# SayanoAI/Comfy-RVC

Hardware: AMD Instinct MI355X
Metric: audio-sec/wall-sec (xRT), 40k_v2 end-to-end VC (higher is better)
Workload: dtype f32; 1 GPU; Full VC 40k_v2 (HuBERT -> RMVPE -> SynthesizerTrnMs768NSFsid), 30 s 16 kHz clips, 12 per GPU per step (3 in flight), vc_single host array in -> int16 host array out (BASELINE.json configs[2]); clips_in_flight_per_gpu=3, weights=procedural (comfy-rvc_amd/synthetic.py), noise=device generator, seeded per clip, parallelism=clip-per-GPU x1 (3 lanes each), one RCCL gather of the step's int16 waveforms

## Files before the change

### comfy-rvc_amd/_lib.py

```python
import ctypes as C
import os

_HERE = os.path.dirname(os.path.abspath(__file__))
LIB_PATH = os.environ.get("RVC_HIP_LIB") or os.path.join(_HERE, "csrc", "librvc_hip.so")


class RvcHipError(RuntimeError):
    pass


def _load():
    if not os.path.isfile(LIB_PATH):
        raise RvcHipError(
            f"{LIB_PATH} is missing: build it with `python -c 'import __graft_entry__ as g; g.build()'` "
            "(or `make -C comfy-rvc_amd/csrc`).  There is no CPU fallback.")
    return C.CDLL(LIB_PATH)


lib = _load()

c_void_p, c_int, c_int64, c_float, c_char_p = C.c_void_p, C.c_int, C.c_int64, C.c_float, C.c_char_p
P = C.POINTER


# ... 148 lines not shown
    "rvc_spectrogram_batch_ms": (c_int, [c_void_p, c_void_p, c_void_p, c_int64, c_void_p, c_int, c_int, c_int, c_float, c_int, c_void_p, c_int64]),
    "rvc_multiscale_mel_loss": (c_int, [c_void_p, c_void_p, c_int, P(c_void_p), P(c_int64), P(c_int64), c_int, c_int64, P(C.c_int32), P(C.c_int32), c_int, c_int,
                                        c_void_p]),
    "rvc_hpss": (c_int, [c_void_p, c_void_p, c_int, c_int, c_int, c_void_p, c_void_p, c_int]),
    "rvc_hpss_l1": (c_int, [c_void_p, c_void_p, c_void_p, c_int, c_int, c_int, c_float, c_void_p]),
    "rvc_tsi_terms": (c_int, [c_void_p, c_void_p, c_void_p, c_int, c_int, c_int, c_float, c_void_p]),
    "rvc_op_gemm_split": (c_int, [c_void_p] * 7 + [c_int] * 4 + [c_float, c_int, c_float] + [c_int] * 5),
    "rvc_op_conv2d_split": (c_int, [c_void_p] * 7 + [c_int] * 9),
    "rvc_op_wn_in_gate_split": (c_int, [c_void_p] * 6 + [c_int] * 4),
    "rvc_op_gemm_split_qkv": (c_int, [c_void_p] * 6 + [c_int] * 4),
    "rvc_op_conv1d_s2_split": (c_int, [c_void_p] * 6 + [c_int] * 5),
    "rvc_op_conv1d_split": (c_int, [c_void_p] * 6 + [c_int] * 9),
    "rvc_op_conv1d": (c_int, [c_void_p, c_void_p, c_void_p, c_void_p, c_void_p, c_void_p] + [c_int] * 8 +
                      [c_int, c_float, c_int, c_float, c_int, c_float, c_int]),
    "rvc_op_conv_transpose1d": (c_int, [c_void_p, c_void_p, c_void_p, c_void_p, c_void_p] + [c_int] * 6 + [c_int, c_float, c_int]),
    "rvc_op_conv2d3x3": (c_int, [c_void_p, c_void_p, c_void_p, c_void_p, c_void_p, c_void_p] + [c_int] * 5),
    "rvc_op_conv_transpose2d": (c_int, [c_void_p, c_void_p, c_void_p, c_void_p, c_void_p] + [c_int] * 5),
    "rvc_op_gemm_tn": (c_int, [c_void_p, c_void_p, c_void_p, c_void_p] + [c_int] * 4),
    "rvc_conv1d_plan_create": (c_int, [c_void_p, c_void_p] + [c_int] * 7 + [P(c_void_p)]),
    "rvc_conv1d_plan_run": (c_int, [c_void_p, c_void_p, c_void_p, c_int, c_void_p, c_void_p, c_int, c_float, c_int, c_float]),
    "rvc_conv1d_plan_pair_run": (c_int, [c_void_p, c_void_p, c_void_p, c_void_p, c_int, c_void_p, c_float, c_int]),
    "rvc_conv1d_plan_resblock_run": (c_int, [P(c_void_p), c_void_p, c_void_p, c_int, c_void_p, c_float, c_int, P(c_int), c_void_p, c_void_p, c_void_p]),
    "rvc_conv1d_plan_pair_split_run": (c_int, [c_void_p, c_void_p, c_void_p, c_void_p, c_int, c_void_p, c_float, c_int]),
    "rvc_conv1d_plan_destroy": (c_int, [c_void_p]),
    "rvc_op_attention": (c_int, [c_void_p, c_void_p, c_void_p, c_void_p, c_void_p, c_void_p, c_int, c_int]),
    "rvc_op_attention_split": (c_int, [c_void_p] * 7 + [c_int, c_int]),
    "rvc_op_attention_split_rel": (c_int, [c_void_p] * 9 + [c_int, c_int, c_int]),
    "rvc_op_cbr2_small": (c_int, [c_void_p] * 7 + [c_int, c_int, c_int]),
    "rvc_op_layernorm_c_split": (c_int, [c_void_p] * 6 + [c_int, c_int]),
    "rvc_op_conv3_small": (c_int, [c_void_p] * 7 + [c_int] * 6),
# ... 100 lines not shown
```

### comfy-rvc_amd/csrc/conv_kernels.h

```cpp
#pragma once
#include "rvc_internal.h"
#include <hip/hip_ext.h>

namespace rvc {

typedef float f32x16 __attribute__((ext_vector_type(16)));
typedef unsigned int u32x4 __attribute__((ext_vector_type(4)));

struct ConvArgsX : ConvArgs {
  long long ldW;
  int Wcols;
  int Wrows;
  int ksplit; float* partial; long long ldP;
  unsigned magRP, magPW;
  int ni; unsigned magNI;
  const unsigned char* Wx; int CoPx; int xbufs; int NC; int kreal; long long wxBatch;
  const unsigned char* Wx2; const float* bias1; int fuse_p2; float fuse_slope;
  const unsigned char* Xs; long long xsTp;
  unsigned char* Ys; long long ysTp; float ys_slope;
  int wbufs;
  int xcd_remap;
  int h2;
};

__device__ __forceinline__ __amdgpu_buffer_rsrc_t make_rsrc(const void* base, unsigned bytes) {
  return __builtin_amdgcn_make_buffer_rsrc(const_cast<void*>(base), 0, (int)bytes, 0x00020000);
}
constexpr unsigned kOOB = 0x80000000u;
__device__ __forceinline__ float buf_load(__amdgpu_buffer_rsrc_t r, unsigned voff, unsigned soff = 0) {
  return __uint_as_float(__builtin_amdgcn_raw_buffer_load_b32(r, (int)voff, (int)soff, 0));
}
__device__ __forceinline__ void buf_dma(__amdgpu_buffer_rsrc_t rs, unsigned char* lds_dst, int voffset, int soffset) {
  __builtin_amdgcn_raw_ptr_buffer_load_lds(rs, (__attribute__((address_space(3))) void*)lds_dst, 16, voffset, soffset, 0, 0);
}

template <int WM, int WN, int AM, int AN, int G, bool HAS_R, bool HAS_ACC>
__device__ __forceinline__ void dense_epilogue_t(const ConvArgsX& p, f32x16 (&acc)[AM][AN], int z, int co0, int n0, int wm, int wn, int li, int lh) {
// ... 104 lines not shown
  dim3 grid; size_t lds = 0;
  int prof_cfg = 0, prof_fused = 0;
  double alg_bytes = 0.0, flops = 0.0;
};
bool conv_x3_plan(const ConvArgsX& a0, int batch, long long Tplan, ConvPlan& p);
void conv_plan_launch(const ConvPlan& p, hipStream_t s);
bool conv_x3p_plan(ConvPlan& p, int AM, int AN);
int conv_x3p_check_read();
bool conv_x3q_plan(ConvPlan& p, int AM, int AN);
bool conv_x3g_plan(ConvPlan& p);
bool conv_x3pf_plan(ConvPlan& p);
bool conv_rbh_plan(ConvPlan& p);
bool conv_x3_pair_plan(const ConvLayer& c1, const ConvLayer& c2, const float* X, long long ldX, int T, long long Tplan, float* Y, long long ldY,
                       const ConvEpilogue& e2, int h2, ConvPlan& p);

struct Rb3Args {
  const float* X; long long ldX; float* Y; long long ldY;
  const unsigned char* W[6];
  const float* B[6];
  int CoPx;
  int T, halo, NO;
  float pre_slope, mid_slope, out_scale;
  const float* nsrc; const float* nw; const float* nb;
};
struct Rb3Plan {
  Rb3Args a; void (*launch)(const Rb3Args&, dim3, size_t, hipStream_t) = nullptr; dim3 grid; size_t lds = 0;
  int C = 0, k = 0, accumulate = 0;
};
bool conv_rb3_plan(const ConvLayer* const* c1, const ConvLayer* const* c2, const float* X, long long ldX, int T, long long Tplan, float* Y, long long ldY,
                   float pre_slope, float out_scale, int accumulate, int h2, const float* nsrc, const float* nw, const float* nb, Rb3Plan& p);
// ... 4 lines not shown
```

### comfy-rvc_amd/csrc/conv_mfma.hip

```cpp
#include "conv_kernels.h"
#include "phase_timing.h"
#include <atomic>
#include <tuple>

#ifndef RVC_EPI_TWOPHASE
#define RVC_EPI_TWOPHASE 0
#endif

namespace rvc {

RVC_PHASE_TABLE_REGISTER;

constexpr int kWSlots = 32;
__host__ __device__ constexpr int x_slots(int BN, int MODE) {
  return MODE == 2 ? (BN >= 512 ? 26 : (BN >= 256 ? 18 : 14)) : (BN >= 512 ? 36 : (BN >= 256 ? 20 : (BN >= 128 ? 32 : 16)));
}

template <int WM, int WN, int AM, int AN, int MODE>
__global__ __launch_bounds__(256) void conv_mfma_kernel(const ConvArgsX p) {
  constexpr int BM = WM * AM * 32, BN = WN * AN * 32;
  constexpr int XS = x_slots(BN, MODE);
  extern __shared__ __attribute__((aligned(16))) float smem[];
  const int CK = p.CK, WROW = p.WROW;
  float* Xs = smem;
// ... 504 lines not shown
          const int u = tap / stride, r = tap % stride;
          const int vc = ci * stride + r;
          const int chunk = vc / L.CK, vcc = vc % L.CK;
          P[(size_t)g * L.wBatch + (((size_t)chunk * L.ktaps + u) * L.CK + vcc) * L.CoP + co] =
              w[((size_t)(g * Cog + co) * Cig + ci) * k + tap];
        }
  upload_layer(L, P, bias, Co);
  if ((g_precision == 2 || (g_precision == 1 && g_x3_default)) && groups == 1 && Ci % 16 == 0 && Co >= 32) {
    pack_x3(L, w, Co, Ci, k);
    if (stride == 1 && Ci == Co && (k == 3 || k == 7 || k == 11) && ((Co % 64 == 0 && Ci >= 64) || Co == 32) && pad == dil * (k - 1) / 2) pack_h2(L, w, Co, Ci, k);
  }
  if ((g_precision == 2 || (g_precision == 1 && g_x3_default)) && groups > 1 && stride == 1 && Cig % 16 == 0 && Cog % 16 == 0 && dil >= 1)
    pack_x3_grouped(L, w, groups, Cog, Cig, k);
}

void tconv1d_layer_init(ConvLayer& L, const float* w, const float* bias, int Ci, int Co, int k, int u, int pad) {
  const int E2 = (k - 1 - pad) / u, E1 = (u - 1 + pad) / u;
  L.mode = 1; L.groups = 1; L.Ci = Ci; L.co_real = Co; L.Co = u * Co; L.CoP = (L.Co + 31) & ~31;
  L.k = E1 + E2 + 1; L.stride = 1; L.dil = 1; L.pad = E2; L.tconv_u = u; L.up2 = 0;
  L.ktaps = L.k;
  L.CK = pick_ck(Ci, L.ktaps, 1);
  L.nchunk = (Ci + L.CK - 1) / L.CK;
  L.wBatch = (long long)L.nchunk * L.ktaps * L.CK * L.CoP;
  std::vector<float> P((size_t)L.wBatch, 0.f);
  for (int r = 0; r < u; ++r)
    for (int co = 0; co < Co; ++co)
      for (int ci = 0; ci < Ci; ++ci)
        for (int j = 0; j < L.ktaps; ++j) {
          const int e = E2 - j;
          const int kk = e * u + r + pad;
          if (kk < 0 || kk >= k) continue;
          const int chunk = ci / L.CK, vcc = ci % L.CK;
          P[(((size_t)chunk * L.ktaps + j) * L.CK + vcc) * L.CoP + (size_t)co * u + r] = w[((size_t)ci * Co + co) * k + kk];
        }
  if ((g_precision == 2 || (g_precision == 1 && g_x3_default)) && Ci % 16 == 0 && L.Co >= 32) {
    std::vector<float> Weq((size_t)L.Co * Ci * L.ktaps, 0.f);
    for (int r = 0; r < u; ++r)
      for (int co = 0; co < Co; ++co)
        for (int ci = 0; ci < Ci; ++ci)
          for (int j = 0; j < L.ktaps; ++j) {
            const int kk = (E2 - j) * u + r + pad;
            if (kk >= 0 && kk < k) Weq[(((size_t)co * u + r) * Ci + ci) * L.ktaps + j] = w[((size_t)ci * Co + co) * k + kk];
          }
    pack_x3(L, Weq.data(), L.Co, Ci, L.ktaps);
  }
  L.k = k; L.pad = pad;
  L.dil = 1;
  L.conv_pad = E2;
  upload_layer(L, P, bias, Co);
}

void conv2d_kx_layer_init(ConvLayer& L, const float* w, const float* bias, int Co, int Ci, int KH, int KW, int PH, int PWL) {
  RVC_REQUIRE(Ci % 16 == 0 && KH >= 1 && KW >= 1 && PH >= 0 && PH < KH && PWL >= 0 && PWL < KW, "conv2d_kx: Ci must be a multiple of 16, padding inside the window");
  L.mode = 2; L.groups = 1; L.Ci = Ci; L.Co = Co; L.co_real = Co; L.CoP = (Co + 31) & ~31;
  L.k = KH * KW; L.stride = 1; L.dil = 1; L.pad = 0; L.tconv_u = 0; L.up2 = 0; L.ktaps = KH * KW;
  L.kh = KH; L.kw = KW; L.ph = PH; L.pwl = PWL;
  L.CK = 16; L.nchunk = Ci / 16; L.wBatch = 0;
  pack_x3(L, w, Co, Ci, KH * KW);
  L.bd_ = bias ? dev_upload(bias, Co) : nullptr;
}
// ... 147 lines not shown
  ProfRec r{t.a, t.b, flops, cfg, bytes, 0, 0, 0, 0, 0, 0, 0, 1, fused, blocks, 0};
  if (a) { r.h2 = a->h2; r.Ci = a->Ci; r.Co = a->Co; r.k = a->kreal > 0 ? a->kreal : a->ktaps; r.dil = a->dil; r.stride = a->stride; r.Tout = a->Tout; r.Wd = a->Wd; r.ksplit = a->ksplit > 0 ? a->ksplit : 1; }
  std::lock_guard<std::mutex> lk(g_prof_mu);
  g_prof.push_back(r);
}
int conv_prof_dump_csv(const char* path) {
  std::lock_guard<std::mutex> lk(g_prof_mu);
  FILE* f = fopen(path, "w");
  if (!f) return -1;
  fprintf(f, "launch,kernel,tile,Ci,Co,k,dil,stride,Tout,Wd,fused_pair,ksplit,workgroups,us,alg_gflop,alg_mbytes,tflops,alg_gbps,mfma_per_product\n");
  int i = 0;
  for (auto& r : g_prof) {
    (void)hipEventSynchronize(r.b);
    float t = 0.f;
    if (hipEventElapsedTime(&t, r.a, r.b) != hipSuccess) continue;
    static const char* kX3Fam[8] = {"conv_x3_kernel", "conv_x3p_kernel", "conv_x3g_kernel", "conv_x3pf_kernel", "conv_x3s_kernel", "conv_rbh_kernel", "conv_x3q_kernel", "conv_rb3_kernel"};
    fprintf(f, "%d,%s,%s,%d,%d,%d,%d,%d,%d,%d,%d,%d,%lld,%.2f,%.4f,%.3f,%.2f,%.1f,%d\n", i++, r.cfg >= 14 ? kX3Fam[(r.fused >> 4) & 7] : "conv_mfma_kernel", kCfgNames[r.cfg],
            r.Ci, r.Co, r.k, r.dil, r.stride, r.Tout, r.Wd, r.fused & 15, r.ksplit, r.blocks, t * 1e3, r.flops / 1e9, r.bytes / 1e6,
            t > 0 ? r.flops / t / 1e9 : 0.0, t > 0 ? r.bytes / t / 1e6 : 0.0, r.cfg >= 14 ? (r.h2 ? 2 : 3) : 1);
  }
  fclose(f);
  return i;
}
double conv_alg_bytes(const ConvArgsX& a, int batch) {
  const double in = (double)a.Ci * (a.Wd > 0 ? (double)a.Tin * a.Wd : (double)a.Tin);
  const double out = (double)a.Co * a.Tout;
  const double w = (double)a.Co * a.Ci * (a.kreal > 0 ? a.kreal : a.ktaps);
  const bool r_is_x = a.R != nullptr && a.R == a.X;
  return 4.0 * (batch * (in + out * (1.0 + ((a.R && !r_is_x) ? 1.0 : 0.0) + (a.accumulate ? 1.0 : 0.0))) + w);
}
int conv_prof_collect_ex(double* out, double ridge_fp32, double ridge_x3) {
  std::lock_guard<std::mutex> lk(g_prof_mu);
// ... 119 lines not shown
static void fill_epilogue(ConvArgsX& a, const ConvEpilogue& e) {
  a.R = e.R; a.ldR = e.ldR; a.pre_act = e.pre_act; a.pre_slope = e.pre_slope; a.act = e.act; a.act_slope = e.act_slope;
  a.act_before_res = e.act_before_res; a.out_scale = e.out_scale; a.accumulate = e.accumulate;
  a.Xs = e.xs_in; a.xsTp = e.xs_tp; a.Ys = e.ys_out; a.ysTp = e.ys_tp; a.ys_slope = e.ys_slope;
}

int conv1d_out_len(const ConvLayer& L, int Tin) {
  if (L.tconv_u > 0) return (Tin - 1) * L.tconv_u - 2 * L.pad + L.k;
  return (Tin + 2 * L.pad - L.dil * (L.k - 1) - 1) / L.stride + 1;
}

void conv1d_run(const ConvLayer& L, hipStream_t s, const float* X, long long ldX, int Tin, float* Y, long long ldY,
                const ConvEpilogue& e0) {
  RVC_REQUIRE(L.mode == 1 && L.Wd_, "conv1d_run on an uninitialised / non-1D layer");
  bool post; const ConvEpilogue e = split_epilogue(e0, post);
  ConvArgsX a{};
  a.X = X; a.W = L.Wd_; a.bias = L.bd_; a.Y = Y;
  fill_epilogue(a, e);
  a.Ci = L.Ci; a.Co = L.Co; a.CoP = L.CoP; a.Tin = Tin; a.Wd = 0; a.ktaps = L.ktaps; a.dil = L.dil; a.stride = L.stride;
  a.CK = L.CK; a.nchunk = L.nchunk;
  a.ldX = ldX; a.ldY = ldY; a.up2 = 0;
  a.ldW = L.CoP; a.Wcols = L.CoP; a.Wrows = L.nchunk * L.ktaps * L.CK;
  if (e.bias_override) a.bias = e.bias_override;
  int Tout = conv1d_out_len(L, Tin);
  if (e.tout_limit > 0 && e.tout_limit < Tout) { RVC_REQUIRE(L.tconv_u == 0, "tout_limit on a transposed conv"); Tout = e.tout_limit; }
  auto gemm_cols = [&](int tout) { return L.tconv_u > 0 ? (tout + L.tconv_u - 1) / L.tconv_u : tout; };
  a.Tout = gemm_cols(Tout);
  RVC_REQUIRE(e.plan_tin == 0 || (e.plan_tin >= Tin && !e.tout_limit), "plan_tin is the input length of the whole sequence this launch is a column window of");
  const long long Tplan = e.plan_tin > 0 ? gemm_cols(conv1d_out_len(L, e.plan_tin)) : a.Tout;
  if (L.tconv_u > 0) {
// ... 104 lines not shown
```

### comfy-rvc_amd/csrc/model_synth.hip

```cpp
#include "model_encoder.h"
#include "models.h"
#include "conv_kernels.h"

namespace rvc {

static OwnedConvLayer make_conv1d(const TensorStore& ts, const std::string& p, int stride, int pad, int dil, bool wn, bool bias = true,
                             float wscale = 1.f, int row0 = 0, int rows = -1) {
  std::vector<float> w; std::vector<long long> shape;
  if (wn) { const HostTensor& v = ts.get(p + ".weight_v"); w = weight_norm0(v, ts.get(p + ".weight_g")); shape = v.shape; }
  else { const HostTensor& v = ts.get(p + ".weight"); w = v.data; shape = v.shape; }
  RVC_REQUIRE(shape.size() == 3, p + ": expected a [Co][Ci][k] weight");
  int Co = (int)shape[0], Ci = (int)shape[1], k = (int)shape[2];
  std::vector<float> b;
  if (bias) b = ts.get(p + ".bias").data;
  if (rows < 0) rows = Co;
  const size_t per = (size_t)Ci * k;
  std::vector<float> ws(w.begin() + row0 * per, w.begin() + (size_t)(row0 + rows) * per);
  if (wscale != 1.f) for (auto& x : ws) x *= wscale;
  std::vector<float> bs;
  if (bias) { bs.assign(b.begin() + row0, b.begin() + row0 + rows); if (wscale != 1.f) for (auto& x : bs) x *= wscale; }
  OwnedConvLayer L;
  conv1d_layer_init(L, ws.data(), bias ? bs.data() : nullptr, rows, Ci, k, stride, pad, dil, 1);
  return L;
}
// ... 394 lines not shown
  for (int i = 0; i < nu; ++i) {
    GenStage& st = S->stages[i];
    const int Cc = S->up_init >> (i + 1);
    const int Tn = Tc * st.u, Tfull_n = Tfull_c * st.u;
    float* up = A.alloc<float>((size_t)Cc * Tn);
    float* t1 = A.alloc<float>((size_t)Cc * Tn);
    float* ya = A.alloc<float>((size_t)Cc * Tn);
    float* yb = A.alloc<float>((size_t)Cc * Tn);
    float* xs = A.alloc<float>((size_t)Cc * Tn);
    float* fr = (S->f0 && st.noise_k > 1) ? A.alloc<float>((size_t)st.noise_k * Tn) : nullptr;
    const GenPairs gp = gen_stage_pairs(st, Tfull_n, h2);
    unsigned char* t1s = gp.any_split ? A.alloc<unsigned char>(split_image_bytes(Cc, Tn)) : nullptr;
    if (!dry) {
      RVC_REQUIRE(conv1d_out_len(st.up, Tc) == Tn, "ConvTranspose1d geometry must give T_out = u * T_in");
      ConvEpilogue Eu; Eu.plan_tin = plan_tin(Tfull_c); Eu.pre_act = ACT_LRELU; Eu.pre_slope = 0.1f;
      conv1d_run(st.up, s, cur, Tc, Tc, up, Tn, Eu);
      ConvEpilogue En; En.plan_tin = plan_tin(Tfull_n); En.accumulate = 1;
      bool noise_in_rb3 = S->f0 && st.noise_k == 1 && st.noise_w.p != nullptr && Nw == (long long)Tn && !(taps && i == 0);
      Rb3Plan rb3[3]; bool rb3_ok[3];
      auto plan_rb3 = [&](bool noise) {
        bool all = true;
        for (int j = 0; j < 3; ++j) {
          const ConvLayer* r1[3] = {&st.rb[j].c1[0], &st.rb[j].c1[1], &st.rb[j].c1[2]};
          const ConvLayer* r2[3] = {&st.rb[j].c2[0], &st.rb[j].c2[1], &st.rb[j].c2[2]};
          rb3_ok[j] = conv_rb3_plan(r1, r2, up, Tn, Tn, Tfull_n, xs, Tn, 0.1f, 1.f / 3.f, j > 0, h2, noise ? har_w : nullptr, noise ? st.noise_w.p : nullptr,
                                    noise ? st.noise_b.p : nullptr, rb3[j]);
          all = all && rb3_ok[j];
        }
        return all;
      };
      if (!plan_rb3(noise_in_rb3) && noise_in_rb3) { noise_in_rb3 = false; plan_rb3(false); }
      if (noise_in_rb3) {
      } else if (!S->f0) {
      } else if (st.noise_w.p && noise_add(s, up, Tn, Cc, Tn, har_w, Nw, st.noise_k, st.noise_s, st.noise_k > 1 ? st.noise_s / 2 : 0, st.noise_w.p, st.noise_b.p)) {
      } else if (st.noise_k > 1) {
        frames(s, har_w, fr, (int)Nw, st.noise_k, st.noise_s, st.noise_s / 2, Tn, 0);
        conv1d_run(st.noise, s, fr, Tn, Tn, up, Tn, En);
      } else {
        conv1d_run(st.noise, s, har_w, Tn, Tn, up, Tn, En);
      }
      if (taps && i == 0) tap(A, s, taps->gen_ups0, up, (size_t)Cc * Tn);
      for (int j = 0; j < 3; ++j) {
        const float* in = up;
        if (rb3_ok[j]) { conv_rb3_launch(rb3[j], s); continue; }
        for (int m = 0; m < 3; ++m) {
          ConvEpilogue E2; E2.plan_tin = plan_tin(Tfull_n); E2.pre_act = ACT_LRELU; E2.pre_slope = 0.1f; E2.R = in; E2.ldR = Tn;
          float* dst = (m == 0) ? ya : (m == 1 ? yb : xs);
// ... 221 lines not shown
```

### comfy-rvc_amd/csrc/rvc_api.hip

```cpp
#include "models.h"
#include "conv_kernels.h"

namespace rvc {
static thread_local std::string g_err;
void set_error(const std::string& msg) { g_err = msg; }
}

using namespace rvc;

struct rvc_ctx { Ctx c; };
static std::mutex g_ctx_mu;
static std::map<int, int> g_ctx_count;
struct rvc_hubert { Hubert* m; rvc_ctx* ctx; };
struct rvc_rmvpe { Rmvpe* m; rvc_ctx* ctx; };
struct rvc_synth { Synth* m; rvc_ctx* ctx; };
struct rvc_conv1d_plan { OwnedConvLayer L; };

#define RVC_TRY try {
#define RVC_CATCH                                                            \
  return 0;                                                                  \
  }                                                                          \
  catch (const std::exception& e) { rvc::set_error(e.what()); return 1; }    \
  catch (...) { rvc::set_error("unknown error"); return 2; }

// ... 967 lines not shown
  }
  check_launch();
  RVC_HIP_CHECK(hipStreamSynchronize(s));
  RVC_CATCH
}
int rvc_op_conv_transpose1d(void* stream, const float* x, const float* w, const float* bias, float* y, int Ci, int Co, int Tin, int k, int u,
                            int pad, int pre_act, float pre_slope, int accumulate) {
  RVC_TRY
  OwnedConvLayer L;
  tconv1d_layer_init(L, w, bias, Ci, Co, k, u, pad);
  ConvEpilogue e; e.pre_act = pre_act; e.pre_slope = pre_slope; e.accumulate = accumulate;
  const int Tout = conv1d_out_len(L, Tin);
  conv1d_run(L, (hipStream_t)stream, x, Tin, Tin, y, Tout, e);
  check_launch();
  RVC_HIP_CHECK(hipStreamSynchronize((hipStream_t)stream));
  RVC_CATCH
}
int rvc_op_conv2d3x3(void* stream, const float* x, const float* w, const float* bias, const float* res, float* y, int Ci, int Co, int H, int W,
                     int relu) {
  RVC_TRY
  OwnedConvLayer L;
  conv2d3x3_layer_init(L, w, bias, Co, Ci);
  ConvEpilogue e; e.act = relu ? ACT_RELU : ACT_NONE; e.act_before_res = 1; e.R = res; e.ldR = (long long)H * W;
  conv2d_run(L, (hipStream_t)stream, x, (long long)H * W, H, W, y, (long long)H * W, e);
  check_launch();
  RVC_HIP_CHECK(hipStreamSynchronize((hipStream_t)stream));
  RVC_CATCH
}
int rvc_op_conv_transpose2d(void* stream, const float* x, const float* w, const float* bias, float* y, int Ci, int Co, int H, int W, int relu) {
  RVC_TRY
// ... 386 lines not shown
```

### comfy-rvc_amd/csrc/rvc_internal.h

```cpp
#pragma once
#include <atomic>
#include <hip/hip_runtime.h>
#include <cstdint>
#include <cstdio>
#include <cstdlib>
#include <cmath>
#include <cstring>
#include <map>
#include <mutex>
#include <string>
#include <vector>
#include <stdexcept>

namespace rvc {

void set_error(const std::string& msg);
struct Error : std::runtime_error { using std::runtime_error::runtime_error; };

#define RVC_HIP_CHECK(expr)                                                                       \
  do {                                                                                            \
    hipError_t _e = (expr);                                                                       \
    if (_e != hipSuccess)                                                                         \
      throw rvc::Error(std::string(#expr) + " failed: " + hipGetErrorString(_e) + " (" + __FILE__ + \
                       ":" + std::to_string(__LINE__) + ")");                                     \
// ... 46 lines not shown
  float* bd_ = nullptr;
  float* bd4_ = nullptr;
  int mode = 1;
  int Ci = 0, Co = 0, CoP = 0, groups = 1;
  int k = 1, stride = 1, dil = 1, pad = 0;
  int ktaps = 1, CK = 8, KT = 1, nchunk = 1;
  int tconv_u = 0;
  int co_real = 0;
  int up2 = 0;
  int conv_pad = 0;
  long long wBatch = 0;
  int kh = 3, kw = 3, ph = 1, pwl = 1;
  uint16_t* Wx_ = nullptr;
  int CoPx = 0; long long wxBatch = 0;
  uint16_t* Wh_ = nullptr;
  int seg2_chunks = 0;
};

struct ConvEpilogue {
  const float* R = nullptr; long long ldR = 0;
  int pre_act = ACT_NONE; float pre_slope = 0.f;
  int act = ACT_NONE; float act_slope = 0.f;
  int act_before_res = 0;
  float out_scale = 1.f; int accumulate = 0;
  const float* bias_override = nullptr;
  int tout_limit = 0;
  int plan_tin = 0;
  const unsigned char* xs_in = nullptr; long long xs_tp = 0;
  unsigned char* ys_out = nullptr; long long ys_tp = 0; float ys_slope = 1.f;
  unsigned char* vt_out = nullptr; long long vt_tp = 0; int vt_row0 = 0;
  int gate_h = 0; const float* gate_g = nullptr;
  int ys_deint_h = 0;
  int h2 = 0;
};
constexpr int kSplitMargin = 64;
inline long long split_image_tp(long long T) { return (T + kSplitMargin + 704 + 63) & ~63LL; }
inline size_t split_image_bytes(int C, long long T) { return (size_t)(C / 16) * 2 * (size_t)split_image_tp(T) * 32; }
enum SplitRole : int { SPLIT_CONSUMER = 0, SPLIT_PRODUCER = 1 };
bool conv1d_split_eligible(const ConvLayer& L, int Tin, SplitRole role = SPLIT_CONSUMER, int h2 = 0);
bool conv1d_pair_h2_eligible(const ConvLayer& c1, const ConvLayer& c2, int Tin, int h2);
int conv1d_residual_period(const ConvLayer& L, int Tin, int h2);
int conv_set_pair_arithmetic(int mode);


void conv1d_layer_init(ConvLayer& L, const float* w , const float* bias, int Co, int Ci, int k,
                       int stride, int pad, int dil, int groups);
void tconv1d_layer_init(ConvLayer& L, const float* w , const float* bias, int Ci, int Co, int k, int u, int pad);
void conv2d3x3_layer_init(ConvLayer& L, const float* w , const float* bias, int Co, int Ci);
// ... 108 lines not shown
  T* get() const { return p; }
  void reset() { dev_free(p); p = nullptr; n = 0; }
  void alloc(size_t cnt) { reset(); p = static_cast<T*>(dev_alloc(cnt * sizeof(T))); n = cnt; }
  void upload(const T* h, size_t cnt) { reset(); p = dev_upload(h, cnt); n = cnt; }
  void upload(const std::vector<T>& h) { upload(h.data(), h.size()); }
};

struct OwnedConvLayer : ConvLayer {
  OwnedConvLayer() = default;
  ~OwnedConvLayer() { free_weights(); }
  OwnedConvLayer(OwnedConvLayer&& o) noexcept : ConvLayer(o) { o.disown(); }
  OwnedConvLayer& operator=(OwnedConvLayer&& o) noexcept { if (this != &o) { free_weights(); ConvLayer::operator=(o); o.disown(); } return *this; }
  OwnedConvLayer(const OwnedConvLayer&) = delete; OwnedConvLayer& operator=(const OwnedConvLayer&) = delete;
  OwnedConvLayer(const ConvLayer&) = delete; OwnedConvLayer& operator=(const ConvLayer&) = delete;
 private:
  void disown() { Wd_ = bd_ = bd4_ = nullptr; Wx_ = Wh_ = nullptr; }
  void free_weights() { dev_free(Wd_); dev_free(bd_); dev_free(bd4_); dev_free(Wx_); dev_free(Wh_); }
};

#define RVC_ALLOW_BIG_LDS(kern)                                                                                                              \
  do {                                                                                                                                       \
    static std::atomic<unsigned long long> rvc_lds_mask_[4];                                                                                 \
    int rvc_dev_ = 0; (void)hipGetDevice(&rvc_dev_);                                                                                         \
    const unsigned long long rvc_bit_ = 1ull << (rvc_dev_ & 63);                                                                             \
    std::atomic<unsigned long long>& rvc_m_ = rvc_lds_mask_[(rvc_dev_ >> 6) & 3];                                                            \
    if (!(rvc_m_.load(std::memory_order_acquire) & rvc_bit_)) {                                                                              \
      RVC_HIP_CHECK(hipFuncSetAttribute(reinterpret_cast<const void*>(kern), hipFuncAttributeMaxDynamicSharedMemorySize, 160 * 1024));      \
      rvc_m_.fetch_or(rvc_bit_, std::memory_order_release);                                                                                  \
    }                                                                                                                                        \
  } while (0)

struct Arena {
// ... 40 lines not shown
```

### include/rvc_hip.h

```cpp
#ifndef RVC_HIP_H
#define RVC_HIP_H
#include <stdint.h>

#ifdef __cplusplus
extern "C" {
#endif

typedef struct rvc_ctx rvc_ctx;
typedef struct rvc_hubert rvc_hubert;
typedef struct rvc_rmvpe rvc_rmvpe;
typedef struct rvc_synth rvc_synth;

const char* rvc_last_error(void);
const char* rvc_version(void);

int rvc_ctx_create(int device_id, rvc_ctx** out);
int rvc_ctx_destroy(rvc_ctx* ctx);
int64_t rvc_ctx_workspace_bytes(rvc_ctx* ctx);
int rvc_ctx_set_conv_precision(rvc_ctx* ctx, int mode);

typedef struct rvc_hubert_taps {
  float* conv_stack;
  float* pos_conv;
  float* hidden_0;
// ... 199 lines not shown

int rvc_op_conv1d(void* stream, const float* x_dev, const float* w_host, const float* bias_host, const float* res_dev, float* y_dev,
                  int Ci, int Co, int Tin, int k, int stride, int pad, int dil, int groups, int pre_act, float pre_slope, int act,
                  float act_slope, int act_before_res, float out_scale, int accumulate);
int rvc_op_gemm_split(void* stream, const float* x_dev, const float* w_host, const float* bias_host, const float* res_dev, float* y_dev,
                      float* ysplit_f32_dev, int Ci, int Co, int T, int act, float act_slope, int act_before_res, float out_scale, int ksplit,
                      int am, int an, int k, int dil);
int rvc_op_conv1d_split(void* stream, const float* x_dev, const float* w_host, const float* bias_host, const float* res_dev, float* y_dev,
                        int Ci, int Co, int T, int k, int pad, int dil, int groups, int act, int act_before_res);
int rvc_op_conv1d_s2_split(void* stream, const float* x_dev, const float* w_host, const float* bias_host, float* y_dev, float* y_img_f32_dev, int Ci, int Co, int T, int k,
                           int act);
int rvc_op_conv2d_split(void* stream, const float* x_dev, const float* w_host, const float* bias_host, const float* res_dev, float* y_dev,
                        float* ysplit_f32_dev, int Ci, int Co, int H, int W, int act, int act_before_res, int ksplit, int am, int an);
int rvc_op_conv_transpose1d(void* stream, const float* x_dev, const float* w_host, const float* bias_host, float* y_dev, int Ci, int Co,
                            int Tin, int k, int u, int pad, int pre_act, float pre_slope, int accumulate);
int rvc_op_conv2d3x3(void* stream, const float* x_dev, const float* w_host, const float* bias_host, const float* res_dev, float* y_dev,
                     int Ci, int Co, int H, int W, int relu);
int rvc_op_conv_transpose2d(void* stream, const float* x_dev, const float* w_host, const float* bias_host, float* y_dev, int Ci, int Co,
                            int H, int W, int relu);
int rvc_op_gemm_tn(void* stream, const float* a_dev, const float* b_dev, float* y_dev, int M, int N, int K, int batch);
typedef struct rvc_conv1d_plan rvc_conv1d_plan;
int rvc_conv1d_plan_create(const float* w_host, const float* bias_host, int Ci, int Co, int k, int stride, int pad, int dil, int groups,
                           rvc_conv1d_plan** out);
int rvc_conv1d_plan_run(rvc_conv1d_plan* p, void* stream, const float* x_dev, int Tin, const float* res_dev, float* y_dev, int pre_act,
                        float pre_slope, int act, float act_slope);
int rvc_conv1d_plan_pair_split_run(rvc_conv1d_plan* c1, rvc_conv1d_plan* c2, void* stream, const float* x_dev, int T, float* y_dev,
                                   float out_scale, int accumulate);
int rvc_conv1d_plan_pair_run(rvc_conv1d_plan* c1, rvc_conv1d_plan* c2, void* stream, const float* x_dev, int T, float* y_dev, float out_scale,
                             int accumulate);
int rvc_conv1d_plan_resblock_run(rvc_conv1d_plan* const* plans6, void* stream, const float* x_dev, int T, float* y_dev, float out_scale, int accumulate,
// ... 71 lines not shown
```

Before: 2413 audio-sec/wall-sec.

## Add tap-major transposed-conv kernel with fused noise-conv epilogue for NSF upsamplers

Adds conv_tup_kernel, which computes ConvTranspose1d as a tap-major GEMM (every output channel times every tap against the input) using bf16-split MFMA. Results go to LDS and are then overlap-added into the u-strided output with bias. The epilogue can also fold in the harmonic-source noise conv (up to 8 taps), so the separate noise_add pass and its extra read-modify-write of the upsampled tensor are gone whenever the resblock path does not already absorb the noise. This replaces the polyphase equivalent-weight conv, which does redundant zero-tap work. The cost is an extra packed weight image per layer, heuristic grid and pass grouping, and a planner that declines some shapes (AM==1 with many tiles), which then fall back.

```diff
diff --git a/comfy-rvc_amd/_lib.py b/comfy-rvc_amd/_lib.py
--- a/comfy-rvc_amd/_lib.py
+++ b/comfy-rvc_amd/_lib.py
@@ -186,6 +186,8 @@
     "rvc_op_conv1d": (c_int, [c_void_p, c_void_p, c_void_p, c_void_p, c_void_p, c_void_p] + [c_int] * 8 +
                       [c_int, c_float, c_int, c_float, c_int, c_float, c_int]),
     "rvc_op_conv_transpose1d": (c_int, [c_void_p, c_void_p, c_void_p, c_void_p, c_void_p] + [c_int] * 6 + [c_int, c_float, c_int]),
+    "rvc_op_conv_transpose1d_noise": (c_int, [c_void_p, c_void_p, c_void_p, c_void_p, c_void_p] + [c_int] * 6 + [c_int, c_float, c_int] + [c_int, c_int] +
+                                      [c_void_p, c_int64, c_int, c_int, c_int, c_void_p, c_void_p, P(c_int)]),
     "rvc_op_conv2d3x3": (c_int, [c_void_p, c_void_p, c_void_p, c_void_p, c_void_p, c_void_p] + [c_int] * 5),
     "rvc_op_conv_transpose2d": (c_int, [c_void_p, c_void_p, c_void_p, c_void_p, c_void_p] + [c_int] * 5),
     "rvc_op_gemm_tn": (c_int, [c_void_p, c_void_p, c_void_p, c_void_p] + [c_int] * 4),
diff --git a/comfy-rvc_amd/csrc/conv_kernels.h b/comfy-rvc_amd/csrc/conv_kernels.h
--- a/comfy-rvc_amd/csrc/conv_kernels.h
+++ b/comfy-rvc_amd/csrc/conv_kernels.h
@@ -21,6 +21,8 @@
   int wbufs;
   int xcd_remap;
   int h2;
+  const unsigned char* Wt; int tupMP, tupCB, tupNP, tupPPG, tk, tpad;
+  const float* nsrc; const float* nw; const float* nb; long long nL; int nk, ns, npad;
 };
 
 __device__ __forceinline__ __amdgpu_buffer_rsrc_t make_rsrc(const void* base, unsigned bytes) {
@@ -155,6 +157,9 @@
 bool conv_x3_pair_plan(const ConvLayer& c1, const ConvLayer& c2, const float* X, long long ldX, int T, long long Tplan, float* Y, long long ldY,
                        const ConvEpilogue& e2, int h2, ConvPlan& p);
 
+bool conv_tup_plan(const ConvLayer& L, const float* X, long long ldX, int Tin, float* Y, long long ldY, const ConvEpilogue& e, ConvPlan& p);
+bool conv_tup_geometry(int Ci, int Co, int k, int u, int pad, int& AM, int& CB);
+
 struct Rb3Args {
   const float* X; long long ldX; float* Y; long long ldY;
   const unsigned char* W[6];
diff --git a/comfy-rvc_amd/csrc/conv_mfma.hip b/comfy-rvc_amd/csrc/conv_mfma.hip
--- a/comfy-rvc_amd/csrc/conv_mfma.hip
+++ b/comfy-rvc_amd/csrc/conv_mfma.hip
@@ -542,6 +542,22 @@
     pack_x3_grouped(L, w, groups, Cog, Cig, k);
 }
 
+static void pack_tup(ConvLayer& L, const float* w , int Ci, int Co, int k, int u, int pad) {
+  int AM = 0, CB = 0;
+  if (!conv_tup_geometry(Ci, Co, k, u, pad, AM, CB)) return;
+  const int PR = 128 * AM, NP = (Co + CB - 1) / CB, MP = NP * PR;
+  std::vector<float> Wr((size_t)MP * Ci, 0.f);
+  for (int co = 0; co < Co; ++co)
+    for (int kk = 0; kk < k; ++kk) {
+      float* row = Wr.data() + ((size_t)(co / CB) * PR + (size_t)(co % CB) * k + kk) * Ci;
+      for (int ci = 0; ci < Ci; ++ci) row[ci] = w[((size_t)ci * Co + co) * k + kk];
+    }
+  std::vector<uint16_t> P;
+  x3_weight_image(Wr.data(), MP, Ci, 1, MP, P);
+  RVC_HIP_CHECK(hipMalloc(&L.Wt_, P.size() * sizeof(uint16_t)));
+  RVC_HIP_CHECK(hipMemcpy(L.Wt_, P.data(), P.size() * sizeof(uint16_t), hipMemcpyHostToDevice));
+  L.tupMP = MP; L.tupAM = AM; L.tupCB = CB;
+}
 void tconv1d_layer_init(ConvLayer& L, const float* w, const float* bias, int Ci, int Co, int k, int u, int pad) {
   const int E2 = (k - 1 - pad) / u, E1 = (u - 1 + pad) / u;
   L.mode = 1; L.groups = 1; L.Ci = Ci; L.co_real = Co; L.Co = u * Co; L.CoP = (L.Co + 31) & ~31;
@@ -572,6 +588,7 @@
           }
     pack_x3(L, Weq.data(), L.Co, Ci, L.ktaps);
   }
+  if ((g_precision == 2 || (g_precision == 1 && g_x3_default)) && Ci % 16 == 0) pack_tup(L, w, Ci, Co, k, u, pad);
   L.k = k; L.pad = pad;
   L.dil = 1;
   L.conv_pad = E2;
@@ -749,8 +766,9 @@
     (void)hipEventSynchronize(r.b);
     float t = 0.f;
     if (hipEventElapsedTime(&t, r.a, r.b) != hipSuccess) continue;
-    static const char* kX3Fam[8] = {"conv_x3_kernel", "conv_x3p_kernel", "conv_x3g_kernel", "conv_x3pf_kernel", "conv_x3s_kernel", "conv_rbh_kernel", "conv_x3q_kernel", "conv_rb3_kernel"};
-    fprintf(f, "%d,%s,%s,%d,%d,%d,%d,%d,%d,%d,%d,%d,%lld,%.2f,%.4f,%.3f,%.2f,%.1f,%d\n", i++, r.cfg >= 14 ? kX3Fam[(r.fused >> 4) & 7] : "conv_mfma_kernel", kCfgNames[r.cfg],
+    static const char* kX3Fam[16] = {"conv_x3_kernel", "conv_x3p_kernel", "conv_x3g_kernel", "conv_x3pf_kernel", "conv_x3s_kernel", "conv_rbh_kernel", "conv_x3q_kernel", "conv_rb3_kernel",
+                                     "conv_tup_kernel", "?", "?", "?", "?", "?", "?", "?"};
+    fprintf(f, "%d,%s,%s,%d,%d,%d,%d,%d,%d,%d,%d,%d,%lld,%.2f,%.4f,%.3f,%.2f,%.1f,%d\n", i++, r.cfg >= 14 ? kX3Fam[(r.fused >> 4) & 15] : "conv_mfma_kernel", kCfgNames[r.cfg],
             r.Ci, r.Co, r.k, r.dil, r.stride, r.Tout, r.Wd, r.fused & 15, r.ksplit, r.blocks, t * 1e3, r.flops / 1e9, r.bytes / 1e6,
             t > 0 ? r.flops / t / 1e9 : 0.0, t > 0 ? r.bytes / t / 1e6 : 0.0, r.cfg >= 14 ? (r.h2 ? 2 : 3) : 1);
   }
@@ -900,6 +918,11 @@
                 const ConvEpilogue& e0) {
   RVC_REQUIRE(L.mode == 1 && L.Wd_, "conv1d_run on an uninitialised / non-1D layer");
   bool post; const ConvEpilogue e = split_epilogue(e0, post);
+  if (L.tconv_u > 0 && L.Wt_) {
+    ConvPlan pt;
+    if (conv_tup_plan(L, X, ldX, Tin, Y, ldY, e, pt)) { conv_plan_launch(pt, s); return; }
+  }
+  RVC_REQUIRE(!e.noise_src, "the noise term is conv_tup_kernel's alone (ask conv_tup_plan before passing it)");
   ConvArgsX a{};
   a.X = X; a.W = L.Wd_; a.bias = L.bd_; a.Y = Y;
   fill_epilogue(a, e);
diff --git a/comfy-rvc_amd/csrc/conv_tup.hip b/comfy-rvc_amd/csrc/conv_tup.hip
--- /dev/null
+++ b/comfy-rvc_amd/csrc/conv_tup.hip
@@ -0,0 +1,267 @@
+#include "conv_x3_dev.h"
+
+namespace rvc {
+
+constexpr int kTupBN = 64;
+constexpr int kTupNQ = kTupBN - 2;
+constexpr int kTupPitch = kTupBN + 1;
+
+template <int AM>
+__global__ __launch_bounds__(256, AM == 1 ? 3 : 1) void conv_tup_kernel(const ConvArgsX p) {
+  constexpr int AN = 2, PR = 128 * AM;
+  typedef float f32x4_t __attribute__((ext_vector_type(4)));
+  extern __shared__ __attribute__((aligned(1024))) unsigned char smem_tup[];
+  const int nck = p.nchunk;
+  unsigned char* Xs = smem_tup;
+  float* S = reinterpret_cast<float*>(smem_tup + (size_t)nck * 4096);
+  float* E = S + PR * kTupPitch;
+
+  const int tid = threadIdx.x, lane = tid & 63;
+  const int wave = __builtin_amdgcn_readfirstlane(tid >> 6);
+  const int li = lane & 31, lh = lane >> 5;
+  const int k = p.tk, u = p.ostride, pad = p.tpad;
+  const int Q0 = (int)blockIdx.x * kTupNQ;
+
+  const long long plane = (long long)p.tupMP * 16;
+  const int pass0 = (int)blockIdx.y * p.tupPPG, pass1 = min(pass0 + p.tupPPG, p.tupNP);
+  auto wrow = [&](int pass) { return p.Wt + (long long)lh * plane + ((long long)pass * PR + wave * (AM * 32) + li) * 16; };
+  const unsigned char* wbase = wrow(pass0);
+  u32x4 ah0[AM], al0[AM], ah1[AM], al1[AM], ah2[AM], al2[AM], ah3[AM], al3[AM];
+  auto load_a = [&](int c, u32x4 (&h)[AM], u32x4 (&l)[AM]) {
+    const unsigned char* w = wbase + (long long)c * 4 * plane;
+#pragma unroll
+    for (int am = 0; am < AM; ++am) {
+      h[am] = *reinterpret_cast<const u32x4*>(w + am * 512);
+      l[am] = *reinterpret_cast<const u32x4*>(w + 2 * plane + am * 512);
+    }
+  };
+  auto load_first = [&]() {
+    load_a(0, ah0, al0); load_a(min(1, nck - 1), ah1, al1); load_a(min(2, nck - 1), ah2, al2); load_a(min(3, nck - 1), ah3, al3);
+  };
+  load_first();
+  {
+    const int CBt = p.tupCB, c0 = pass0 * CBt, nch = min(p.tupPPG * CBt, p.Co - c0);
+    for (int i = tid; i < nch * 10; i += 256) {
+      const int c = i / 10, f = i - c * 10, co = c0 + c;
+      float v = 0.f;
+      if (f == 0) v = p.bias ? p.bias[co] : 0.f;
+      else if (p.nsrc) v = f == 1 ? p.nb[co] : (f - 2 < p.nk ? p.nw[co * p.nk + f - 2] : 0.f);
+      E[i] = v;
+    }
+  }
+
+  {
+    const float pre_slope = p.pre_act == ACT_LRELU ? p.pre_slope : 1.f;
+    const __amdgpu_buffer_rsrc_t xrs = make_rsrc(p.X, (unsigned)p.Ci * (unsigned)p.ldX * 4u);
+    const int q = Q0 - 1 + lane;
+    const unsigned voff = (q >= 0 && q < p.Tin) ? (unsigned)q * 4u : kOOB;
+    const int nslot = 2 * nck;
+    for (int s0 = wave; s0 < nslot; s0 += 16) {
+      float xr[4][8];
+#pragma unroll
+      for (int i = 0; i < 4; ++i) {
+        const int s = s0 + 4 * i;
+#pragma unroll
+        for (int j = 0; j < 8; ++j) xr[i][j] = buf_load(xrs, s < nslot ? voff : kOOB, s < nslot ? (unsigned)(s * 8 + j) * (unsigned)p.ldX * 4u : 0u);
+      }
+#pragma unroll
+      for (int i = 0; i < 4; ++i) {
+        const int s = s0 + 4 * i;
+        if (s < nslot) {
+          u32x4 hi, lo;
+#pragma unroll
+          for (int j = 0; j < 4; ++j) {
+            const float a = xr[i][2 * j], b = xr[i][2 * j + 1];
+            unsigned h_, l_;
+            split2(fmaxf(a, a * pre_slope), fmaxf(b, b * pre_slope), h_, l_);
+            hi[j] = h_; lo[j] = l_;
+          }
+          unsigned char* d = Xs + (s >> 1) * 4096 + (s & 1) * 1024 + lane * 16;
+          *reinterpret_cast<u32x4*>(d) = hi;
+          *reinterpret_cast<u32x4*>(d + 2048) = lo;
+        }
+      }
+    }
+  }
+  __syncthreads();
+
+  const int CB = p.tupCB;
+  const int t0 = Q0 * u;
+  const int nt = min(kTupNQ * u, p.Tout - t0);
+  const bool vec = (p.ldY & 3) == 0 && (reinterpret_cast<uintptr_t>(p.Y) & 15) == 0 && (t0 & 3) == 0;
+  const unsigned char* xa = Xs + lh * 1024 + li * 16;
+
+  const int nq4 = (kTupNQ * u + 3) >> 2;
+  const int NG = 256 / nq4;
+  const int j4 = tid % nq4, cg = tid / nq4, tl = 4 * j4;
+  const bool live = cg < NG && tl < nt;
+  int so[4][3];
+  float sv[4][8];
+  {
+    int Ql = tl / u, r = tl - Ql * u;
+#pragma unroll
+    for (int e = 0; e < 4; ++e) {
+      const int kc = r + pad;
+      const bool in = live && tl + e < nt;
+      so[e][0] = (in && kc + u < k) ? (kc + u) * kTupPitch + Ql : -1;
+      so[e][1] = (in && kc < k) ? kc * kTupPitch + Ql + 1 : -1;
+      so[e][2] = (in && kc >= u) ? (kc - u) * kTupPitch + Ql + 2 : -1;
+      const long long p0 = (long long)(t0 + tl + e) * p.ns - p.npad;
+#pragma unroll
+      for (int j = 0; j < 8; ++j) {
+        const long long qn = p0 + j;
+        sv[e][j] = (p.nsrc && in && j < p.nk && qn >= 0 && qn < p.nL) ? p.nsrc[qn] : 0.f;
+      }
+      if (++r == u) { r = 0; ++Ql; }
+    }
+  }
+
+  for (int pass = pass0; pass < pass1; ++pass) {
+    f32x16 acc[AM][AN];
+#pragma unroll
+    for (int am = 0; am < AM; ++am)
+#pragma unroll
+      for (int an = 0; an < AN; ++an)
+#pragma unroll
+        for (int r = 0; r < 16; ++r) acc[am][an][r] = 0.f;
+
+    auto mac = [&](int c, const u32x4 (&h)[AM], const u32x4 (&l)[AM]) {
+      u32x4 bh[AN], bl[AN];
+#pragma unroll
+      for (int an = 0; an < AN; ++an) {
+        bl[an] = *reinterpret_cast<const u32x4*>(xa + c * 4096 + 2048 + an * 512);
+        bh[an] = *reinterpret_cast<const u32x4*>(xa + c * 4096 + an * 512);
+      }
+#pragma unroll
+      for (int am = 0; am < AM; ++am)
+#pragma unroll
+        for (int an = 0; an < AN; ++an)
+          acc[am][an] = __builtin_amdgcn_mfma_f32_32x32x16_bf16(__builtin_bit_cast(bf16x8, h[am]), __builtin_bit_cast(bf16x8, bl[an]), acc[am][an], 0, 0, 0);
+#pragma unroll
+      for (int am = 0; am < AM; ++am)
+#pragma unroll
+        for (int an = 0; an < AN; ++an)
+          acc[am][an] = __builtin_amdgcn_mfma_f32_32x32x16_bf16(__builtin_bit_cast(bf16x8, l[am]), __builtin_bit_cast(bf16x8, bh[an]), acc[am][an], 0, 0, 0);
+#pragma unroll
+      for (int am = 0; am < AM; ++am)
+#pragma unroll
+        for (int an = 0; an < AN; ++an)
+          acc[am][an] = __builtin_amdgcn_mfma_f32_32x32x16_bf16(__builtin_bit_cast(bf16x8, h[am]), __builtin_bit_cast(bf16x8, bh[an]), acc[am][an], 0, 0, 0);
+    };
+    for (int c = 0; c < nck; c += 4) {
+      mac(c, ah0, al0);
+      if (c + 4 < nck) load_a(c + 4, ah0, al0);
+      if (c + 1 < nck) { mac(c + 1, ah1, al1); if (c + 5 < nck) load_a(c + 5, ah1, al1); }
+      if (c + 2 < nck) { mac(c + 2, ah2, al2); if (c + 6 < nck) load_a(c + 6, ah2, al2); }
+      if (c + 3 < nck) { mac(c + 3, ah3, al3); if (c + 7 < nck) load_a(c + 7, ah3, al3); }
+    }
+
+    if (pass + 1 < pass1) { wbase = wrow(pass + 1); load_first(); }
+
+#pragma unroll
+    for (int am = 0; am < AM; ++am)
+#pragma unroll
+      for (int an = 0; an < AN; ++an)
+#pragma unroll
+        for (int r = 0; r < 16; ++r)
+          S[(wave * (AM * 32) + am * 32 + (r & 3) + 8 * (r >> 2) + 4 * lh) * kTupPitch + an * 32 + li] = acc[am][an][r];
+    __syncthreads();
+
+    for (int cl = live ? cg : CB; cl < CB; cl += NG) {
+      const int co = pass * CB + cl;
+      if (co >= p.Co) break;
+      const float* Sc = S + cl * k * kTupPitch;
+      const float* Ec = E + ((pass - pass0) * CB + cl) * 10;
+      const float bv = Ec[0];
+      float nwc[8], nbc = 0.f;
+      if (p.nsrc) {
+        nbc = Ec[1];
+#pragma unroll
+        for (int j = 0; j < 8; ++j) nwc[j] = Ec[2 + j];
+      }
+      float v[4];
+#pragma unroll
+      for (int e = 0; e < 4; ++e) {
+        const float s0 = Sc[max(so[e][0], 0)], s1 = Sc[max(so[e][1], 0)], s2 = Sc[max(so[e][2], 0)];
+        float a = so[e][0] >= 0 ? s0 : 0.f;
+        a += so[e][1] >= 0 ? s1 : 0.f;
+        a += so[e][2] >= 0 ? s2 : 0.f;
+        a += bv;
+        if (p.nsrc) {
+          float n = nbc;
+#pragma unroll
+          for (int j = 0; j < 8; ++j)
+            if (j < p.nk) n = fmaf(nwc[j], sv[e][j], n);
+          a += n;
+        }
+        v[e] = a;
+      }
+      float* yp = p.Y + (long long)co * p.ldY + t0 + tl;
+      if (vec && tl + 3 < nt) {
+        f32x4_t o = {v[0], v[1], v[2], v[3]};
+        if (p.accumulate) o += *reinterpret_cast<const f32x4_t*>(yp);
+        *reinterpret_cast<f32x4_t*>(yp) = o;
+      } else {
+#pragma unroll
+        for (int e = 0; e < 4; ++e)
+          if (tl + e < nt) yp[e] = p.accumulate ? v[e] + yp[e] : v[e];
+      }
+    }
+    __syncthreads();
+  }
+}
+
+template <int AM>
+static void launch_tup(const ConvArgsX& a, dim3 grid, size_t lds, hipStream_t s) {
+  auto kern = conv_tup_kernel<AM>;
+  RVC_ALLOW_BIG_LDS(kern);
+  conv_launch(kern, grid, dim3(256), lds, s, a);
+}
+
+static size_t tup_lds_bytes(int Ci, int AM, int chans) { return (size_t)(Ci / 16) * 4096 + (size_t)128 * AM * kTupPitch * sizeof(float) + (size_t)chans * 40; }
+
+bool conv_tup_geometry(int Ci, int Co, int k, int u, int pad, int& AM, int& CB) {
+  if (Ci <= 0 || (Ci & 15) || Co <= 0 || u < 1 || u > 16 || pad < 0 || pad > u || k < 1 || k > 3 * u || k - 1 - pad >= 2 * u) return false;
+  AM = (long long)Co * k >= 1024 ? 2 : 1;
+  if (k > 128 * AM) return false;
+  CB = 128 * AM / k;
+  return tup_lds_bytes(Ci, AM, Co + 128 * AM) <= 160 * 1024;
+}
+
+bool conv_tup_plan(const ConvLayer& L, const float* X, long long ldX, int Tin, float* Y, long long ldY, const ConvEpilogue& e, ConvPlan& p) {
+  if (!L.Wt_ || L.tconv_u <= 0 || L.mode != 1 || e.tup_off) return false;
+  if (e.R || e.act != ACT_NONE || e.out_scale != 1.f || e.xs_in || e.ys_out || e.h2 || e.tout_limit || !(e.pre_act == ACT_NONE || e.pre_act == ACT_LRELU)) return false;
+  const int Tout = conv1d_out_len(L, Tin);
+  if (Tin <= 0 || Tout <= 0 || ldY < Tout || ldX < Tin || (double)L.Ci * (double)ldX * 4.0 >= 2147483648.0) return false;
+  if (e.noise_src && (e.noise_k < 1 || e.noise_k > 8 || !e.noise_w || !e.noise_b || e.accumulate)) return false;
+  const int u = L.tconv_u, AM = L.tupAM, CB = L.tupCB;
+  const int NP = (L.co_real + CB - 1) / CB;
+  const long long Tplan = e.plan_tin > 0 ? conv1d_out_len(L, e.plan_tin) : Tout;
+  const long long tiles_plan = ((Tplan + u - 1) / u + kTupNQ - 1) / kTupNQ;
+  if (AM == 1 && tiles_plan >= 4LL * device_cu_count()) return false;
+  int G = 1;
+  while (G < NP && tiles_plan * G < 3LL * device_cu_count()) ++G;
+  const int PPG = (NP + G - 1) / G;
+  G = (NP + PPG - 1) / PPG;
+  p = ConvPlan{};
+  p.plan_T = Tplan;
+  ConvArgsX& a = p.a;
+  a.X = X; a.Y = Y; a.bias = e.bias_override ? e.bias_override : L.bd_;
+  a.Ci = L.Ci; a.Co = L.co_real; a.CoP = L.tupMP; a.Tin = Tin; a.Tout = Tout; a.ldX = ldX; a.ldY = ldY;
+  a.ktaps = L.k; a.kreal = L.k; a.dil = 1; a.stride = 1; a.pad = L.pad; a.CK = 16; a.nchunk = L.Ci / 16;
+  a.pre_act = e.pre_act; a.pre_slope = e.pre_slope; a.act = ACT_NONE; a.out_scale = 1.f; a.accumulate = e.accumulate;
+  a.ostride = u; a.orows = L.co_real; a.ksplit = 1;
+  a.Wt = reinterpret_cast<const unsigned char*>(L.Wt_); a.tupMP = L.tupMP; a.tupCB = CB; a.tupNP = NP; a.tupPPG = PPG; a.tk = L.k; a.tpad = L.pad;
+  if (e.noise_src) { a.nsrc = e.noise_src; a.nw = e.noise_w; a.nb = e.noise_b; a.nL = e.noise_L; a.nk = e.noise_k; a.ns = e.noise_s; a.npad = e.noise_pad; }
+  const long long tiles = (((long long)Tout + u - 1) / u + kTupNQ - 1) / kTupNQ;
+  p.grid = dim3((unsigned)tiles, (unsigned)G, 1);
+  p.lds = tup_lds_bytes(L.Ci, AM, PPG * CB);
+  p.launch = AM == 2 ? &launch_tup<2> : &launch_tup<1>;
+  p.prof_cfg = 14 + (AM == 2 ? 3 : 5);
+  p.prof_fused = 8 << 4;
+  p.flops = 2.0 * Tin * (double)L.Ci * L.co_real * L.k;
+  p.alg_bytes = conv_alg_bytes(a, 1) + (e.noise_src ? 4.0 * (double)e.noise_L : 0.0);
+  return true;
+}
+
+}
diff --git a/comfy-rvc_amd/csrc/model_synth.hip b/comfy-rvc_amd/csrc/model_synth.hip
--- a/comfy-rvc_amd/csrc/model_synth.hip
+++ b/comfy-rvc_amd/csrc/model_synth.hip
@@ -432,7 +432,6 @@
     if (!dry) {
       RVC_REQUIRE(conv1d_out_len(st.up, Tc) == Tn, "ConvTranspose1d geometry must give T_out = u * T_in");
       ConvEpilogue Eu; Eu.plan_tin = plan_tin(Tfull_c); Eu.pre_act = ACT_LRELU; Eu.pre_slope = 0.1f;
-      conv1d_run(st.up, s, cur, Tc, Tc, up, Tn, Eu);
       ConvEpilogue En; En.plan_tin = plan_tin(Tfull_n); En.accumulate = 1;
       bool noise_in_rb3 = S->f0 && st.noise_k == 1 && st.noise_w.p != nullptr && Nw == (long long)Tn && !(taps && i == 0);
       Rb3Plan rb3[3]; bool rb3_ok[3];
@@ -448,7 +447,16 @@
         return all;
       };
       if (!plan_rb3(noise_in_rb3) && noise_in_rb3) { noise_in_rb3 = false; plan_rb3(false); }
-      if (noise_in_rb3) {
+      bool noise_in_up = false;
+      if (!noise_in_rb3 && S->f0 && st.noise_w.p && st.noise_k <= 8) {
+        ConvEpilogue Eun = Eu;
+        Eun.noise_src = har_w; Eun.noise_L = Nw; Eun.noise_k = st.noise_k; Eun.noise_s = st.noise_s; Eun.noise_pad = st.noise_k > 1 ? st.noise_s / 2 : 0;
+        Eun.noise_w = st.noise_w.p; Eun.noise_b = st.noise_b.p;
+        ConvPlan pu;
+        if (conv_tup_plan(st.up, cur, Tc, Tc, up, Tn, Eun, pu)) { conv_plan_launch(pu, s); noise_in_up = true; }
+      }
+      if (!noise_in_up) conv1d_run(st.up, s, cur, Tc, Tc, up, Tn, Eu);
+      if (noise_in_rb3 || noise_in_up) {
       } else if (!S->f0) {
       } else if (st.noise_w.p && noise_add(s, up, Tn, Cc, Tn, har_w, Nw, st.noise_k, st.noise_s, st.noise_k > 1 ? st.noise_s / 2 : 0, st.noise_w.p, st.noise_b.p)) {
       } else if (st.noise_k > 1) {
diff --git a/comfy-rvc_amd/csrc/rvc_api.hip b/comfy-rvc_amd/csrc/rvc_api.hip
--- a/comfy-rvc_amd/csrc/rvc_api.hip
+++ b/comfy-rvc_amd/csrc/rvc_api.hip
@@ -1005,6 +1005,25 @@
   conv1d_run(L, (hipStream_t)stream, x, Tin, Tin, y, Tout, e);
   check_launch();
   RVC_HIP_CHECK(hipStreamSynchronize((hipStream_t)stream));
+  RVC_CATCH
+}
+int rvc_op_conv_transpose1d_noise(void* stream, const float* x, const float* w, const float* bias, float* y, int Ci, int Co, int Tin, int k, int u, int pad,
+                                  int pre_act, float pre_slope, int accumulate, int plan_tin, int polyphase, const float* nsrc, int64_t nL, int nk, int nstride,
+                                  int npad, const float* nw, const float* nb, int* ran_out) {
+  RVC_TRY
+  RVC_REQUIRE(x && w && y && ran_out && Ci > 0 && Co > 0 && Tin > 0, "bad argument");
+  hipStream_t s = (hipStream_t)stream;
+  OwnedConvLayer L;
+  tconv1d_layer_init(L, w, bias, Ci, Co, k, u, pad);
+  ConvEpilogue e; e.pre_act = pre_act; e.pre_slope = pre_slope; e.accumulate = accumulate; e.plan_tin = plan_tin; e.tup_off = polyphase ? 1 : 0;
+  if (nsrc) { e.noise_src = nsrc; e.noise_L = nL; e.noise_k = nk; e.noise_s = nstride; e.noise_pad = npad; e.noise_w = nw; e.noise_b = nb; }
+  const int Tout = conv1d_out_len(L, Tin);
+  ConvPlan p;
+  *ran_out = conv_tup_plan(L, x, Tin, Tin, y, Tout, e, p) ? 1 : 0;
+  RVC_REQUIRE(*ran_out || !nsrc, "the noise term needs the tap-major kernel, and conv_tup_plan declined this layer");
+  conv1d_run(L, s, x, Tin, Tin, y, Tout, e);
+  check_launch();
+  RVC_HIP_CHECK(hipStreamSynchronize(s));
   RVC_CATCH
 }
 int rvc_op_conv2d3x3(void* stream, const float* x, const float* w, const float* bias, const float* res, float* y, int Ci, int Co, int H, int W,
diff --git a/comfy-rvc_amd/csrc/rvc_internal.h b/comfy-rvc_amd/csrc/rvc_internal.h
--- a/comfy-rvc_amd/csrc/rvc_internal.h
+++ b/comfy-rvc_amd/csrc/rvc_internal.h
@@ -84,6 +84,8 @@
   uint16_t* Wx_ = nullptr;
   int CoPx = 0; long long wxBatch = 0;
   uint16_t* Wh_ = nullptr;
+  uint16_t* Wt_ = nullptr;
+  int tupMP = 0, tupAM = 0, tupCB = 0;
   int seg2_chunks = 0;
 };
 
@@ -102,6 +104,8 @@
   int gate_h = 0; const float* gate_g = nullptr;
   int ys_deint_h = 0;
   int h2 = 0;
+  const float* noise_src = nullptr; long long noise_L = 0; int noise_k = 0, noise_s = 1, noise_pad = 0; const float* noise_w = nullptr; const float* noise_b = nullptr;
+  int tup_off = 0;
 };
 constexpr int kSplitMargin = 64;
 inline long long split_image_tp(long long T) { return (T + kSplitMargin + 704 + 63) & ~63LL; }
@@ -240,8 +244,8 @@
   OwnedConvLayer(const OwnedConvLayer&) = delete; OwnedConvLayer& operator=(const OwnedConvLayer&) = delete;
   OwnedConvLayer(const ConvLayer&) = delete; OwnedConvLayer& operator=(const ConvLayer&) = delete;
  private:
-  void disown() { Wd_ = bd_ = bd4_ = nullptr; Wx_ = Wh_ = nullptr; }
-  void free_weights() { dev_free(Wd_); dev_free(bd_); dev_free(bd4_); dev_free(Wx_); dev_free(Wh_); }
+  void disown() { Wd_ = bd_ = bd4_ = nullptr; Wx_ = Wh_ = Wt_ = nullptr; }
+  void free_weights() { dev_free(Wd_); dev_free(bd_); dev_free(bd4_); dev_free(Wx_); dev_free(Wh_); dev_free(Wt_); }
 };
 
 #define RVC_ALLOW_BIG_LDS(kern)                                                                                                              \
diff --git a/include/rvc_hip.h b/include/rvc_hip.h
--- a/include/rvc_hip.h
+++ b/include/rvc_hip.h
@@ -237,6 +237,9 @@
                         float* ysplit_f32_dev, int Ci, int Co, int H, int W, int act, int act_before_res, int ksplit, int am, int an);
 int rvc_op_conv_transpose1d(void* stream, const float* x_dev, const float* w_host, const float* bias_host, float* y_dev, int Ci, int Co,
                             int Tin, int k, int u, int pad, int pre_act, float pre_slope, int accumulate);
+int rvc_op_conv_transpose1d_noise(void* stream, const float* x_dev, const float* w_host, const float* bias_host, float* y_dev, int Ci, int Co, int Tin, int k,
+                                  int u, int pad, int pre_act, float pre_slope, int accumulate, int plan_tin, int polyphase, const float* nsrc_dev, int64_t nL,
+                                  int nk, int nstride, int npad, const float* nw_dev, const float* nb_dev, int* ran_out);
 int rvc_op_conv2d3x3(void* stream, const float* x_dev, const float* w_host, const float* bias_host, const float* res_dev, float* y_dev,
                      int Ci, int Co, int H, int W, int relu);
 int rvc_op_conv_transpose2d(void* stream, const float* x_dev, const float* w_host, const float* bias_host, float* y_dev, int Ci, int Co,
```

After: 2416 audio-sec/wall-sec, median of 3. No clear change (+0.1%).
